# OpenDriveLab/ViDAR

Hardware: AMD Instinct MI355X
Metric: train samples/sec (6-cam->BEV step) (higher is better)
Workload: dtype f32

## Files before the change

### vidar_amd/csrc/dcn.hip

```cpp
#include <hip/hip_runtime.h>
#include <stdint.h>

#include "vidar_hip.h"
#include "vidar_common.h"
#include "det_scatter.h"

namespace {

struct PlaneTile { int plane, tile; bool ok; };
__device__ __forceinline__ PlaneTile xcd_plane_tile(int L, int T, int planes) {
  const int xcd = L & 7, j = L >> 3;
  const int pl = (j / T) * 8 + xcd;
  return PlaneTile{pl, j - (j / T) * T, pl < planes};
}
inline unsigned xcd_plane_grid(int T, int planes) { return 8u * (unsigned)T * (unsigned)((planes + 7) / 8); }

struct Conv { int C, H, W, Ho, Wo, kh, kw, stride, pad, dil; };

struct Bil {
  int h0, w0;
  float lh, lw;
  bool in, t, b, l, r;
};

__device__ __forceinline__ Bil bil(float h, float w, int H, int W) {
  Bil q;
  q.in = h > -1.f && w > -1.f && h < H && w < W;
  q.h0 = (int)floorf(h); q.w0 = (int)floorf(w);
  q.lh = h - q.h0; q.lw = w - q.w0;
  q.t = q.h0 >= 0; q.b = q.h0 + 1 <= H - 1; q.l = q.w0 >= 0; q.r = q.w0 + 1 <= W - 1;
  return q;
}

struct Pos { float h, w; };
__device__ __forceinline__ Pos tap_pos(const Conv& g, int py, int px, int t, float oh, float ow) {
  const int i = t / g.kw, j = t - i * g.kw;
  return Pos{py * g.stride - g.pad + i * g.dil + oh, px * g.stride - g.pad + j * g.dil + ow};
}

template <class F>
__device__ __forceinline__ void for_corners(const Bil& q, int W, F f) {
  const float hh = 1.f - q.lh, hw = 1.f - q.lw;
  const int tl = q.h0 * W + q.w0;
  if (q.t && q.l) f(tl, hh * hw);
  if (q.t && q.r) f(tl + 1, hh * q.lw);
  if (q.b && q.l) f(tl + W, q.lh * hw);
  if (q.b && q.r) f(tl + W + 1, q.lh * q.lw);
}

constexpr int kMaxTaps = 9;

typedef float pair_t __attribute__((ext_vector_type(2), aligned(4)));

template <bool PAIR>
__device__ __forceinline__ pair_t load_pair(const void* p) {
  if constexpr (PAIR) return *reinterpret_cast<const pair_t*>(p);
  else return pair_t{*reinterpret_cast<const float*>(p), 0.f};
}

struct PairMap {
  int top, bot;
  bool same, left;
  __device__ __forceinline__ float e0(float cl, float cr) const { return same ? cl : (left ? cr : 0.f); }
  __device__ __forceinline__ float e1(float cl, float cr) const { return same ? cr : (left ? 0.f : cl); }
};

__device__ __forceinline__ PairMap pair_map(const Bil& q, int H, int W) {
  const int c0 = min(max(q.w0, 0), max(W - 2, 0));
  const int r0 = min(max(q.h0, 0), H - 1), r1 = min(max(q.h0 + 1, 0), H - 1);
  return PairMap{r0 * W + c0, r1 * W + c0, q.w0 == c0, q.w0 < c0};
}

constexpr int kCP = 16;
struct TapFoot { unsigned top, bot; float wt0, wt1, wb0, wb1; };

__device__ __forceinline__ TapFoot tap_foot(Pos s, float m, const Conv& g) {
  const Bil q = bil(s.h, s.w, g.H, g.W);
  const PairMap pm = pair_map(q, g.H, g.W);
  const float wl = (q.l ? 1.f - q.lw : 0.f), wr = (q.r ? q.lw : 0.f);
  const float a0 = pm.e0(wl, wr), a1 = pm.e1(wl, wr);
  const float ht = (q.t ? 1.f - q.lh : 0.f) * m, hb = (q.b ? q.lh : 0.f) * m;
  TapFoot f;
  f.top = (unsigned)pm.top * 4u; f.bot = (unsigned)pm.bot * 4u;
  f.wt0 = q.in ? ht * a0 : 0.f; f.wt1 = q.in ? ht * a1 : 0.f;
  f.wb0 = q.in ? hb * a0 : 0.f; f.wb1 = q.in ? hb * a1 : 0.f;
  return f;
}

template <bool PAIR>
__device__ __forceinline__ void im2col_body(const float* __restrict__ x, const float* __restrict__ offset,
                                            const float* __restrict__ mask, float* __restrict__ cols, const Conv& g, int nimg) {
  const int P = g.Ho * g.Wo, K = g.kh * g.kw;
  const int cgroups = (g.C + kCP - 1) / kCP;
  const PlaneTile pt = xcd_plane_tile(blockIdx.x, (P + 255) / 256, cgroups * nimg);
  if (!pt.ok) return;
  const int p = pt.tile * 256 + threadIdx.x;
  if (p >= P) return;
  const int n = pt.plane / cgroups, c0 = (pt.plane - n * cgroups) * kCP, nc = min(kCP, g.C - c0);
  const int py = p / g.Wo, px = p % g.Wo;
  const size_t plane = (size_t)g.H * g.W, KP = (size_t)K * P;
  const char* im = reinterpret_cast<const char*>(x + ((size_t)n * g.C + c0) * plane);
  float* out = cols + ((size_t)n * g.C + c0) * KP + p;
  const float* off_n = offset + (size_t)n * 2 * K * P + p;
  const float* msk_n = mask + (size_t)n * K * P + p;
  float oh = off_n[0], ow = off_n[P], m = msk_n[0];
  for (int t = 0; t < K; ++t) {
    const TapFoot f = tap_foot(tap_pos(g, py, px, t, oh, ow), m, g);
    pair_t a[kCP], b[kCP];
#pragma unroll
    for (int c = 0; c < kCP; ++c) {
      const char* pl = im + (size_t)(c < nc ? c : 0) * plane * 4;
      a[c] = load_pair<PAIR>(pl + f.top);
      b[c] = load_pair<PAIR>(pl + f.bot);
    }
    if (t + 1 < K) {
      oh = off_n[(size_t)(2 * t + 2) * P]; ow = off_n[(size_t)(2 * t + 3) * P]; m = msk_n[(size_t)(t + 1) * P];
    }
#pragma unroll
    for (int c = 0; c < kCP; ++c)
      if (c < nc) {
        const float v = f.wt0 * a[c].x + f.wt1 * a[c].y + f.wb0 * b[c].x + f.wb1 * b[c].y;
        __builtin_nontemporal_store(v, out + (size_t)c * KP + (size_t)t * P);
      }
  }
}

__global__ __launch_bounds__(256) void dcn_im2col_pair_kernel(
    const float* __restrict__ x, const float* __restrict__ offset, const float* __restrict__ mask,
    float* __restrict__ cols, Conv g, int nimg) {
  im2col_body<true>(x, offset, mask, cols, g, nimg);
}
__global__ __launch_bounds__(256) void dcn_im2col_kernel(
    const float* __restrict__ x, const float* __restrict__ offset, const float* __restrict__ mask,
    float* __restrict__ cols, Conv g, int nimg) {
  im2col_body<false>(x, offset, mask, cols, g, nimg);
}

constexpr int kCG = 8;
template <class Acc>
__global__ __launch_bounds__(256) void dcn_col2im_kernel(const float* __restrict__ grad_cols, const float* __restrict__ offset,
                                                         const float* __restrict__ mask, float* __restrict__ grad_x, Conv g,
                                                         typename Acc::Param param) {
  Acc acc(grad_x, param);
  const int P = g.Ho * g.Wo, K = g.kh * g.kw;
  const int p = blockIdx.x * 256 + threadIdx.x;
  if constexpr (!Acc::kMeasureOnly) {
    if (p >= P) return;
  }
  const int n = blockIdx.z, c0 = blockIdx.y * kCG, nc = min(kCG, g.C - c0);
  const int py = p / g.Wo, px = p % g.Wo;
  const size_t plane = (size_t)g.H * g.W, KP = (size_t)K * P;
  float* gim = grad_x + ((size_t)n * g.C + c0) * plane;
  const float* gc = grad_cols + ((size_t)n * g.C + c0) * KP + p;
  for (int t = 0; t < K; ++t) {
    if constexpr (Acc::kMeasureOnly) {
      if (p >= P) break;
    }
    const size_t o = ((size_t)n * 2 * K + 2 * t) * P + p;
    const Pos s = tap_pos(g, py, px, t, offset[o], offset[o + P]);
    const Bil q = bil(s.h, s.w, g.H, g.W);
    if (!q.in) continue;
    const float m = mask[((size_t)n * K + t) * P + p];
    for (int c = 0; c < nc; ++c) {
      const float gv = gc[(size_t)c * KP + (size_t)t * P] * m;
      if (gv == 0.f) continue;
      for_corners(q, g.W, [&](int pix, float w) { acc.add(gim + (size_t)c * plane + pix, w * gv); });
    }
  }
  acc.flush();
}

struct Entry { int src; float w; };

template <bool FILL>
__global__ __launch_bounds__(256) void dcn_revmap_kernel(const float* __restrict__ offset,
                                                         const float* __restrict__ mask, int* __restrict__ cursor,
                                                         Entry* __restrict__ rec, Conv g) {
  const int P = g.Ho * g.Wo, K = g.kh * g.kw, HW = g.H * g.W;
  const int p = blockIdx.x * 256 + threadIdx.x;
  if (p >= P) return;
  const int t = blockIdx.y, n = blockIdx.z;
  const int py = p / g.Wo, px = p % g.Wo;
  const size_t o = ((size_t)n * 2 * K + 2 * t) * P + p;
  const Pos s = tap_pos(g, py, px, t, offset[o], offset[o + P]);
  const Bil q = bil(s.h, s.w, g.H, g.W);
  if (!q.in) return;
  const float m = FILL ? mask[((size_t)n * K + t) * P + p] : 0.f;
  int* cur = cursor + ((size_t)n * K + t) * HW;
  const int src = t * P + p;
  for_corners(q, g.W, [&](int pix, float w) {
    if (FILL) rec[atomicAdd(cur + pix, 1)] = Entry{src, w * m};
    else atomicAdd(cur + pix, 1);
  });
}

__global__ __launch_bounds__(1024) void dcn_revmap_scan_kernel(int* __restrict__ cursor, int* __restrict__ first,
                                                               int HW, int per_image) {
  __shared__ int s_part[1024];
  const int n = blockIdx.x;
  int* cnt = cursor + (size_t)n * HW;
  int* fst = first + (size_t)n * HW;
  const int per = (HW + 1023) / 1024;
  const int r0 = min(HW, (int)threadIdx.x * per), r1 = min(HW, r0 + per);
  int sum = 0;
  for (int i = r0; i < r1; ++i) sum += cnt[i];
  s_part[threadIdx.x] = sum;
  __syncthreads();
  for (int d = 1; d < 1024; d <<= 1) {
    const int a = (int)threadIdx.x >= d ? s_part[threadIdx.x - d] : 0;
    __syncthreads();
    s_part[threadIdx.x] += a;
    __syncthreads();
  }
  int run = n * per_image + s_part[threadIdx.x] - sum;
  for (int i = r0; i < r1; ++i) { const int c = cnt[i]; fst[i] = run; cnt[i] = run; run += c; }
}

constexpr int kGC = 16;
__global__ __launch_bounds__(256) void dcn_col2im_gather_kernel(const float* __restrict__ grad_cols,
                                                                const int* __restrict__ first,
                                                                const int* __restrict__ last,
                                                                const Entry* __restrict__ rec,
                                                                float* __restrict__ grad_x, Conv g) {
  const int P = g.Ho * g.Wo, K = g.kh * g.kw, HW = g.H * g.W;
  const int pix = blockIdx.x * 256 + threadIdx.x;
  if (pix >= HW) return;
  const int n = blockIdx.z, c0 = blockIdx.y * kGC;
  float acc[kGC];
#pragma unroll
  for (int c = 0; c < kGC; ++c) acc[c] = 0.f;
  const size_t KP = (size_t)K * P;
  const float* gc = grad_cols + ((size_t)n * g.C + c0) * KP;
  const int nc = min(kGC, g.C - c0);
  for (int t = 0; t < K; ++t) {
    const size_t bin = ((size_t)n * K + t) * HW + pix;
    const int e0 = first[bin], e1 = last[bin];
    if (nc == kGC) {
      int e = e0;
      for (; e + 1 < e1; e += 2) {
        const Entry r0 = rec[e], r1 = rec[e + 1];
        float v0[kGC], v1[kGC];
#pragma unroll
        for (int c = 0; c < kGC; ++c) { v0[c] = gc[(size_t)c * KP + r0.src]; v1[c] = gc[(size_t)c * KP + r1.src]; }
#pragma unroll
        for (int c = 0; c < kGC; ++c) acc[c] += r0.w * v0[c] + r1.w * v1[c];
      }
      if (e < e1) {
        const Entry r = rec[e];
#pragma unroll
        for (int c = 0; c < kGC; ++c) acc[c] += r.w * gc[(size_t)c * KP + r.src];
      }
    } else {
      for (int e = e0; e < e1; ++e) {
        const Entry r = rec[e];
        for (int c = 0; c < nc; ++c) acc[c] += r.w * gc[(size_t)c * KP + r.src];
      }
    }
  }
  for (int c = 0; c < nc; ++c) grad_x[((size_t)n * g.C + c0 + c) * HW + pix] = acc[c];
}

#ifndef VIDAR_DCN_GRY
#define VIDAR_DCN_GRY 2
#endif
#ifndef VIDAR_DCN_GLC
#define VIDAR_DCN_GLC 8
#endif
constexpr int kGRY = VIDAR_DCN_GRY;
constexpr int kGTH = 8 * kGRY, kGTW = 32;
#ifndef VIDAR_DCN_GHALO
#define VIDAR_DCN_GHALO 5
#endif
constexpr int kGHalo = VIDAR_DCN_GHALO;
constexpr int kGWH = kGTH + 2 * kGHalo + 2;
constexpr int kGWW = kGTW + 2 * kGHalo + 2;
constexpr int kGWP = (kGWW + 3) / 4 * 4;
constexpr int kGWS = kGWH * kGWP;
constexpr int kGLC = VIDAR_DCN_GLC;
constexpr int kGPos = (kGWS + 255) / 256;

__global__ __launch_bounds__(256) void dcn_col2im_gather_lds_kernel(
    const float* __restrict__ grad_cols, const int* __restrict__ first, const int* __restrict__ last,
    const Entry* __restrict__ rec, float* __restrict__ grad_x, Conv g, int tiles_x, int tiles_y, int nimg, float inv_wo) {
  __shared__ __attribute__((aligned(16))) float s_gc[kGLC * kGWS];
  constexpr int K = 9;
  const int P = g.Ho * g.Wo, HW = g.H * g.W;
  const int cgroups = (g.C + kGLC - 1) / kGLC;
  const PlaneTile pt = xcd_plane_tile(blockIdx.x, tiles_x * tiles_y, cgroups * nimg);
  if (!pt.ok) return;
  const int tile = pt.tile, tyi = tile / tiles_x, txi = tile - tyi * tiles_x;
  const int n = pt.plane / cgroups, c0 = (pt.plane - n * cgroups) * kGLC, nc = min(kGLC, g.C - c0);
  const int ry = threadIdx.x / kGTW, rx = threadIdx.x % kGTW;
  const int dx = txi * kGTW + rx;
  const size_t KP = (size_t)K * P;
  const float* gc = grad_cols + ((size_t)n * g.C + c0) * KP;
  float acc[kGRY][kGLC];
#pragma unroll
  for (int k = 0; k < kGRY; ++k)
#pragma unroll
    for (int c = 0; c < kGLC; ++c) acc[k][c] = 0.f;
  for (int t = 0; t < K; ++t) {
    const int i = t / 3, j = t - i * 3;
    const int wy0 = tyi * kGTH + g.pad - i - kGHalo - 1, wx0 = txi * kGTW + g.pad - j - kGHalo - 1;
    const float* gct = gc + (size_t)t * P;
    __syncthreads();
    {
      const int wave = __builtin_amdgcn_readfirstlane((int)threadIdx.x >> 6);
#pragma unroll
      for (int k = 0; k < kGPos; ++k) {
        const int e = threadIdx.x + k * 256;
        const int r = e / kGWP, cc = e - r * kGWP;
        const int sy = wy0 + r, sx = wx0 + cc;
        const bool ok = e < kGWS && sy >= 0 && sy < g.Ho && sx >= 0 && sx < g.Wo && cc < kGWW;
        const int off = ok ? sy * g.Wo + sx : 0;
        if (ok) {
#pragma unroll
          for (int c = 0; c < kGLC; ++c)
            __builtin_amdgcn_global_load_lds((const __attribute__((address_space(1))) void*)(gct + (size_t)(c < nc ? c : 0) * KP + off),
                                             (__attribute__((address_space(3))) void*)(s_gc + c * kGWS + k * 256 + wave * 64), 4, 0, 0);
        }
      }
    }
    __syncthreads();
    if (dx >= g.W) continue;
#pragma unroll
    for (int k = 0; k < kGRY; ++k) {
      const int dy = tyi * kGTH + ry + 8 * k;
      if (dy >= g.H) continue;
      const size_t bin = ((size_t)n * K + t) * HW + dy * g.W + dx;
      const int e1 = last[bin];
      int e = first[bin];
      Entry nxt = e < e1 ? rec[e] : Entry{0, 0.f};
      while (e < e1) {
        const Entry r = nxt;
        ++e;
        if (e < e1) nxt = rec[e];
        const int p = r.src - t * P;
        const int py = (int)((p + 0.5f) * inv_wo), px = p - py * g.Wo;
        const int ly = py - wy0, lx = px - wx0;
        if (ly >= 0 && ly < kGWH && lx >= 0 && lx < kGWW) {
          const float* q = s_gc + ly * kGWP + lx;
#pragma unroll
          for (int c = 0; c < kGLC; ++c) acc[k][c] += r.w * q[c * kGWS];
        } else {
          for (int c = 0; c < nc; ++c) acc[k][c] += r.w * gct[(size_t)c * KP + p];
        }
      }
    }
  }
  if (dx < g.W) {
#pragma unroll
    for (int k = 0; k < kGRY; ++k) {
      const int dy = tyi * kGTH + ry + 8 * k;
      if (dy < g.H)
        for (int c = 0; c < nc; ++c) grad_x[((size_t)n * g.C + c0 + c) * HW + dy * g.W + dx] = acc[k][c];
    }
  }
}

int g_dcn_variant = 1;

template <bool PAIR>
__device__ __forceinline__ void col2im_coord_body(const float* __restrict__ grad_cols, const float* __restrict__ x,
                                                  const float* __restrict__ offset, const float* __restrict__ mask,
                                                  float* __restrict__ grad_offset, float* __restrict__ grad_mask,
                                                  const Conv& g) {
  const int P = g.Ho * g.Wo, K = g.kh * g.kw;
  const int p = blockIdx.x * 256 + threadIdx.x;
  if (p >= P) return;
  const int t = blockIdx.y, n = blockIdx.z;
  const int py = p / g.Wo, px = p % g.Wo;
  const size_t o = ((size_t)n * 2 * K + 2 * t) * P + p;
  const Pos s = tap_pos(g, py, px, t, offset[o], offset[o + P]);
  const float m = mask[((size_t)n * K + t) * P + p];
  const Bil q = bil(s.h, s.w, g.H, g.W);
  float gh = 0.f, gw = 0.f, gm = 0.f;
  if (q.in) {
    const float hh = 1.f - q.lh, hw = 1.f - q.lw;
    const PairMap pm = pair_map(q, g.H, g.W);
    const float tl = (q.t && q.l) ? 1.f : 0.f, tr = (q.t && q.r) ? 1.f : 0.f;
    const float bl = (q.b && q.l) ? 1.f : 0.f, br = (q.b && q.r) ? 1.f : 0.f;
    const float m_t0 = pm.e0(hh * hw * tl, hh * q.lw * tr), m_t1 = pm.e1(hh * hw * tl, hh * q.lw * tr);
    const float m_b0 = pm.e0(q.lh * hw * bl, q.lh * q.lw * br), m_b1 = pm.e1(q.lh * hw * bl, q.lh * q.lw * br);
    const float h_t0 = pm.e0(-hw * tl, -q.lw * tr), h_t1 = pm.e1(-hw * tl, -q.lw * tr);
    const float h_b0 = pm.e0(hw * bl, q.lw * br), h_b1 = pm.e1(hw * bl, q.lw * br);
    const float w_t0 = pm.e0(-hh * tl, hh * tr), w_t1 = pm.e1(-hh * tl, hh * tr);
    const float w_b0 = pm.e0(-q.lh * bl, q.lh * br), w_b1 = pm.e1(-q.lh * bl, q.lh * br);
    int c = 0;
    constexpr int kCB = 8;
    const unsigned top_b = (unsigned)pm.top * 4u, bot_b = (unsigned)pm.bot * 4u, p_b = (unsigned)p * 4u;
    const size_t plane_b = (size_t)g.H * g.W * 4, col_b = (size_t)K * P * 4;
    for (; c + kCB <= g.C; c += kCB) {
      const char* im0 = reinterpret_cast<const char*>(x) + ((size_t)n * g.C + c) * plane_b;
      const char* gc0 = reinterpret_cast<const char*>(grad_cols) + (((size_t)n * g.C + c) * K + t) * (size_t)P * 4;
      pair_t a[kCB], b[kCB];
      float gc[kCB];
#pragma unroll
      for (int u = 0; u < kCB; ++u) {
        gc[u] = *reinterpret_cast<const float*>(gc0 + u * col_b + p_b);
        a[u] = load_pair<PAIR>(im0 + u * plane_b + top_b);
        b[u] = load_pair<PAIR>(im0 + u * plane_b + bot_b);
      }
      __builtin_amdgcn_sched_barrier(0);
#pragma unroll
      for (int u = 0; u < kCB; ++u) {
        gm += gc[u] * (m_t0 * a[u].x + m_t1 * a[u].y + m_b0 * b[u].x + m_b1 * b[u].y);
        gh += gc[u] * (h_t0 * a[u].x + h_t1 * a[u].y + h_b0 * b[u].x + h_b1 * b[u].y);
        gw += gc[u] * (w_t0 * a[u].x + w_t1 * a[u].y + w_b0 * b[u].x + w_b1 * b[u].y);
      }
    }
    for (; c < g.C; ++c) {
      const float* im = x + ((size_t)n * g.C + c) * g.H * g.W;
      const float gc = grad_cols[(((size_t)n * g.C + c) * K + t) * P + p];
      const pair_t a = load_pair<PAIR>(im + pm.top), b = load_pair<PAIR>(im + pm.bot);
      gm += gc * (m_t0 * a.x + m_t1 * a.y + m_b0 * b.x + m_b1 * b.y);
      gh += gc * (h_t0 * a.x + h_t1 * a.y + h_b0 * b.x + h_b1 * b.y);
      gw += gc * (w_t0 * a.x + w_t1 * a.y + w_b0 * b.x + w_b1 * b.y);
    }
  }
  grad_offset[o] = gh * m;
  grad_offset[o + P] = gw * m;
  grad_mask[((size_t)n * K + t) * P + p] = gm;
}

__global__ __launch_bounds__(256) void dcn_col2im_coord_kernel(
    const float* __restrict__ grad_cols, const float* __restrict__ x, const float* __restrict__ offset,
    const float* __restrict__ mask, float* __restrict__ grad_offset, float* __restrict__ grad_mask, Conv g) {
  col2im_coord_body<true>(grad_cols, x, offset, mask, grad_offset, grad_mask, g);
}
__global__ __launch_bounds__(256) void dcn_col2im_coord_1col_kernel(
    const float* __restrict__ grad_cols, const float* __restrict__ x, const float* __restrict__ offset,
    const float* __restrict__ mask, float* __restrict__ grad_offset, float* __restrict__ grad_mask, Conv g) {
  col2im_coord_body<false>(grad_cols, x, offset, mask, grad_offset, grad_mask, g);
}

inline bool dcn_bad(int N, const Conv& g) {
  return N < 0 || g.C <= 0 || g.H <= 0 || g.W <= 0 || g.Ho <= 0 || g.Wo <= 0 || g.kh <= 0 ||
         g.kw <= 0 || g.stride <= 0 || g.dil <= 0 || g.pad < 0;
}

}

extern "C" {

int vidar_dcn_set_variant(int variant) {
  const int prev = g_dcn_variant;
  if (variant >= 0 && variant <= 1) g_dcn_variant = variant;
  return prev;
}

int vidar_dcn_im2col_f32(const float* x, const float* offset, const float* mask, float* cols, int N,
                         int C, int H, int W, int Ho, int Wo, int kh, int kw, int stride, int pad,
                         int dil, void* stream) {
  VIDAR_ENTER();
  Conv g{C, H, W, Ho, Wo, kh, kw, stride, pad, dil};
  if (dcn_bad(N, g)) return VIDAR_ERR_BAD_ARG;
  if (N == 0) return 0;
  if (kh * kw > kMaxTaps) return VIDAR_ERR_BAD_ARG;
  hipLaunchKernelGGL(W >= 2 ? dcn_im2col_pair_kernel : dcn_im2col_kernel,
                     dim3(xcd_plane_grid((Ho * Wo + 255) / 256, ((C + kCP - 1) / kCP) * N)), dim3(256), 0, (hipStream_t)stream,
                     x, offset, mask, cols, g, N);
  return vidar_last_error();
}

size_t vidar_dcn_col2im_workspace_bytes(int N, int H, int W, int Ho, int Wo, int kh, int kw) {
  if (N <= 0 || H <= 0 || W <= 0 || Ho <= 0 || Wo <= 0 || kh <= 0 || kw <= 0) return 0;
  const size_t hw = (size_t)N * kh * kw * H * W, ent = (size_t)N * kh * kw * Ho * Wo * 4;
  if (ent >= (1ull << 31)) return 0;
  return sizeof(int) * 2 * hw + sizeof(Entry) * ent;
}

int vidar_dcn_col2im_det_workspace_bytes(int N, int C, int H, int W, int64_t* bytes) {
  if (N < 0 || C < 0 || H < 0 || W < 0 || !bytes) return VIDAR_ERR_BAD_ARG;
  *bytes = (int64_t)det_workspace_bytes((size_t)N * C * H * W);
  return 0;
}

int vidar_dcn_col2im_f32(const float* grad_cols, const float* x, const float* offset,
                         const float* mask, float* grad_x, float* grad_offset, float* grad_mask,
                         int N, int C, int H, int W, int Ho, int Wo, int kh, int kw, int stride,
                         int pad, int dil, void* workspace, size_t workspace_bytes, void* stream) {
  VIDAR_ENTER();
  Conv g{C, H, W, Ho, Wo, kh, kw, stride, pad, dil};
  if (dcn_bad(N, g)) return VIDAR_ERR_BAD_ARG;
  hipStream_t s = (hipStream_t)stream;
  if (N == 0) return 0;
  if (kh * kw > kMaxTaps) return VIDAR_ERR_BAD_ARG;
  const int P = Ho * Wo, K = kh * kw, HW = H * W;
  if (det_mode()) {
    const dim3 grid((P + 255) / 256, (C + kCG - 1) / kCG, N);
    const int rc = det_scatter(
        grad_x, nullptr, (size_t)N * C * HW, 0, (uint64_t)N * C * K * P * 4, false, workspace, workspace_bytes, s,
        [&](auto tag, auto param, auto) {
          hipLaunchKernelGGL(dcn_col2im_kernel<decltype(tag)>, grid, dim3(256), 0, s, grad_cols, offset, mask, grad_x, g,
                             param);
        });
    if (rc != 0) return rc;
  } else if (workspace) {
    const size_t need = vidar_dcn_col2im_workspace_bytes(N, H, W, Ho, Wo, kh, kw);
    if (need == 0 || workspace_bytes < need) return VIDAR_ERR_BAD_ARG;
    int* cursor = (int*)workspace;
    int* first = cursor + (size_t)N * K * HW;
    Entry* rec = (Entry*)(first + (size_t)N * K * HW);
    hipError_t e = hipMemsetAsync(cursor, 0, sizeof(int) * (size_t)N * K * HW, s);
    if (e != hipSuccess) return (int)e;
    const dim3 rgrid((P + 255) / 256, K, N);
    hipLaunchKernelGGL(dcn_revmap_kernel<false>, rgrid, dim3(256), 0, s, offset, mask, cursor, rec, g);
    hipLaunchKernelGGL(dcn_revmap_scan_kernel, dim3(N * K), dim3(1024), 0, s, cursor, first, HW, P * 4);
    hipLaunchKernelGGL(dcn_revmap_kernel<true>, rgrid, dim3(256), 0, s, offset, mask, cursor, rec, g);
    if ((g_dcn_variant & 1) && kh == 3 && kw == 3 && stride == 1 && dil == 1 && Ho == H && Wo == W) {
      const int tiles_x = (W + kGTW - 1) / kGTW, tiles_y = (H + kGTH - 1) / kGTH;
      hipLaunchKernelGGL(dcn_col2im_gather_lds_kernel, dim3(xcd_plane_grid(tiles_x * tiles_y, ((C + kGLC - 1) / kGLC) * N)), dim3(256), 0,
                         s, grad_cols, first, cursor, rec, grad_x, g, tiles_x, tiles_y, N, 1.0f / (float)Wo);
    } else {
      hipLaunchKernelGGL(dcn_col2im_gather_kernel, dim3((HW + 255) / 256, (C + kGC - 1) / kGC, N), dim3(256), 0, s,
                         grad_cols, first, cursor, rec, grad_x, g);
    }
  } else {
    hipError_t e = hipMemsetAsync(grad_x, 0, sizeof(float) * (size_t)N * C * H * W, s);
    if (e != hipSuccess) return (int)e;
    hipLaunchKernelGGL(dcn_col2im_kernel<det::AccAtomic>, dim3((P + 255) / 256, (C + kCG - 1) / kCG, N), dim3(256), 0, s, grad_cols,
                       offset, mask, grad_x, g, det::AccAtomic::Param{});
  }
  hipLaunchKernelGGL(W >= 2 ? dcn_col2im_coord_kernel : dcn_col2im_coord_1col_kernel, dim3((P + 255) / 256, K, N), dim3(256), 0,
                     s, grad_cols, x, offset, mask, grad_offset, grad_mask, g);
  return vidar_last_error();
}

}
```

Baseline: 2.940.

## Stage input channel planes in LDS for deformable im2col gather

Adds an im2col kernel that copies whole input channel planes (up to 4 channels) into up to 160KB of LDS using global_load_lds, then does the bilinear gathers from LDS rather than global memory. This is meant to cut scattered global and L2 traffic from the deformable sampling. It becomes the default variant when the planes fit. The trade-off is far fewer, larger 1024-thread workgroups (one per image and channel group), lower occupancy, and a serial staging phase before any sampling starts.

```diff
diff --git a/vidar_amd/csrc/dcn.hip b/vidar_amd/csrc/dcn.hip
--- a/vidar_amd/csrc/dcn.hip
+++ b/vidar_amd/csrc/dcn.hip
@@ -136,6 +136,85 @@
   im2col_body<false>(x, offset, mask, cols, g, nimg);
 }
 
+constexpr size_t kLdsBytes = 160 * 1024;
+
+inline int plane_channels(int want, size_t floats) {
+  const size_t fit = kLdsBytes / (floats * sizeof(float));
+  const int g = (int)(fit < (size_t)want ? fit : (size_t)want);
+  return g >= 2 ? g : 0;
+}
+
+template <typename K>
+inline bool allow_lds(K kernel, size_t bytes) {
+  if (bytes <= 64 * 1024) return true;
+  static const bool ok = hipFuncSetAttribute(reinterpret_cast<const void*>(kernel), hipFuncAttributeMaxDynamicSharedMemorySize,
+                                             (int)kLdsBytes) == hipSuccess;
+  return ok;
+}
+
+__device__ __forceinline__ void stage_floats(const float* __restrict__ src, float* dst, int n) {
+  const int wave0 = __builtin_amdgcn_readfirstlane((int)threadIdx.x & ~63), lane = (int)threadIdx.x & 63;
+  const int vec = __builtin_amdgcn_readfirstlane((int)((((uintptr_t)src | (uintptr_t)dst) & 15) == 0));
+  const int n4 = vec ? n >> 2 : 0;
+  for (int i = wave0; i < n4; i += (int)blockDim.x)
+    if (i + lane < n4)
+      __builtin_amdgcn_global_load_lds((const __attribute__((address_space(1))) void*)(src + 4 * (size_t)(i + lane)),
+                                       (__attribute__((address_space(3))) void*)(dst + 4 * i), 16, 0, 0);
+  for (int i = 4 * n4 + wave0; i < n; i += (int)blockDim.x)
+    if (i + lane < n)
+      __builtin_amdgcn_global_load_lds((const __attribute__((address_space(1))) void*)(src + (size_t)(i + lane)),
+                                       (__attribute__((address_space(3))) void*)(dst + i), 4, 0, 0);
+}
+
+#ifndef VIDAR_DCN_PLANE_G
+#define VIDAR_DCN_PLANE_G 4
+#endif
+#ifndef VIDAR_DCN_PLANE_WG
+#define VIDAR_DCN_PLANE_WG 1024
+#endif
+constexpr int kPG = VIDAR_DCN_PLANE_G;
+constexpr int kPW = VIDAR_DCN_PLANE_WG;
+
+__global__ __launch_bounds__(kPW) void dcn_im2col_plane_kernel(
+    const float* __restrict__ x, const float* __restrict__ offset, const float* __restrict__ mask,
+    float* __restrict__ cols, Conv g, int gch) {
+  extern __shared__ __attribute__((aligned(16))) float s_plane[];
+  const int P = g.Ho * g.Wo, K = g.kh * g.kw, HW = g.H * g.W;
+  const int cgroups = (g.C + gch - 1) / gch;
+  const int n = blockIdx.x / cgroups, c0 = (blockIdx.x - n * cgroups) * gch, nc = min(gch, g.C - c0);
+  stage_floats(x + ((size_t)n * g.C + c0) * HW, s_plane, nc * HW);
+  __syncthreads();
+  const size_t KP = (size_t)K * P;
+  const unsigned plane_b = (unsigned)HW * 4u;
+  for (int p = threadIdx.x; p < P; p += kPW) {
+    const int py = p / g.Wo, px = p - py * g.Wo;
+    float* out = cols + ((size_t)n * g.C + c0) * KP + p;
+    const float* off_n = offset + (size_t)n * 2 * K * P + p;
+    const float* msk_n = mask + (size_t)n * K * P + p;
+    float oh = off_n[0], ow = off_n[P], m = msk_n[0];
+    for (int t = 0; t < K; ++t) {
+      const TapFoot f = tap_foot(tap_pos(g, py, px, t, oh, ow), m, g);
+      if (t + 1 < K) {
+        oh = off_n[(size_t)(2 * t + 2) * P]; ow = off_n[(size_t)(2 * t + 3) * P]; m = msk_n[(size_t)(t + 1) * P];
+      }
+      const char* pl = reinterpret_cast<const char*>(s_plane);
+      pair_t a[kPG], b[kPG];
+#pragma unroll
+      for (int c = 0; c < kPG; ++c) {
+        const unsigned pb = (c < nc ? c : 0) * plane_b;
+        a[c] = load_pair<true>(pl + pb + f.top);
+        b[c] = load_pair<true>(pl + pb + f.bot);
+      }
+#pragma unroll
+      for (int c = 0; c < kPG; ++c)
+        if (c < nc) {
+          const float v = f.wt0 * a[c].x + f.wt1 * a[c].y + f.wb0 * b[c].x + f.wb1 * b[c].y;
+          __builtin_nontemporal_store(v, out + (size_t)c * KP + (size_t)t * P);
+        }
+    }
+  }
+}
+
 constexpr int kCG = 8;
 template <class Acc>
 __global__ __launch_bounds__(256) void dcn_col2im_kernel(const float* __restrict__ grad_cols, const float* __restrict__ offset,
@@ -358,7 +437,7 @@
   }
 }
 
-int g_dcn_variant = 1;
+int g_dcn_variant = 3;
 
 template <bool PAIR>
 __device__ __forceinline__ void col2im_coord_body(const float* __restrict__ grad_cols, const float* __restrict__ x,
@@ -445,7 +524,7 @@
 
 int vidar_dcn_set_variant(int variant) {
   const int prev = g_dcn_variant;
-  if (variant >= 0 && variant <= 1) g_dcn_variant = variant;
+  if (variant >= 0 && variant <= 3) g_dcn_variant = variant;
   return prev;
 }
 
@@ -457,9 +536,17 @@
   if (dcn_bad(N, g)) return VIDAR_ERR_BAD_ARG;
   if (N == 0) return 0;
   if (kh * kw > kMaxTaps) return VIDAR_ERR_BAD_ARG;
-  hipLaunchKernelGGL(W >= 2 ? dcn_im2col_pair_kernel : dcn_im2col_kernel,
-                     dim3(xcd_plane_grid((Ho * Wo + 255) / 256, ((C + kCP - 1) / kCP) * N)), dim3(256), 0, (hipStream_t)stream,
-                     x, offset, mask, cols, g, N);
+  const int fit = (g_dcn_variant & 2) && W >= 2 ? plane_channels(kPG, (size_t)H * W) : 0;
+  const int gch = fit < C ? fit : C;
+  const size_t lds = (size_t)gch * H * W * sizeof(float);
+  if (fit && allow_lds(dcn_im2col_plane_kernel, lds)) {
+    hipLaunchKernelGGL(dcn_im2col_plane_kernel, dim3((unsigned)(N * ((C + gch - 1) / gch))), dim3(kPW), lds, (hipStream_t)stream,
+                       x, offset, mask, cols, g, gch);
+  } else {
+    hipLaunchKernelGGL(W >= 2 ? dcn_im2col_pair_kernel : dcn_im2col_kernel,
+                       dim3(xcd_plane_grid((Ho * Wo + 255) / 256, ((C + kCP - 1) / kCP) * N)), dim3(256), 0, (hipStream_t)stream,
+                       x, offset, mask, cols, g, N);
+  }
   return vidar_last_error();
 }
 
```

New measurement: 2.949 (median of 6 runs). About the same (+0.3%).
